# zju3dv/pvnet

Measured on NVIDIA H100. Metric: images/sec (480x640, K=9) backbone+vote, higher is better.
Workload: dtype tf32 (fp32 storage, fp32 accumulate; vote fp32/fp64)

## Files before the change

pvnet_b200/csrc/conv_col.cu:

```cuda
#include "conv_tc.cuh"
#include "ptx.cuh"

#include <cstdlib>
#include <mutex>
#include <new>

namespace pvnet {

int g_conv_mode = 0;

namespace {

constexpr int COL_TH = 16, COL_TW = 8;
constexpr int COL_THREADS = 384;
constexpr int HEAD_MAX = 64;

__host__ __device__ constexpr int head_pitch(int hc) { return hc <= 8 ? 8 : (hc <= 24 ? 24 : 40); }
constexpr int HEAD_CPITCH = COL_TH * COL_TW + 4;
__host__ __device__ constexpr int head_stage_floats(int hc)
{
    return COL_TH * COL_TW * head_pitch(hc) > hc * HEAD_CPITCH ? COL_TH * COL_TW * head_pitch(hc) : hc * HEAD_CPITCH;
}
__host__ __device__ constexpr int head_stage_bytes(int hc) { return (head_stage_floats(hc) * 4 + COL_TH * COL_TW + 127) & ~127; }

struct ColGeom {
    int Ho, Wo, tiles_x, tiles_y, total_tiles;
    int cin_chunks, cin_pad;
    int split_chunk;
    int pad_l, pad_t;
    int stages;
    int resident;
    int out_cs, out_co, res_cs, res_co;
    int act, round_out;
    int head_cout, head_seg, mask_esz;
    int head_nhwc;
};

__device__ __forceinline__ void head_store_tile(const ColGeom &g, uint32_t sv, uint32_t sm, float *head_out, void *mask,
                                                int img, int y0, int x0, int tid, int nthr)
{
    const int hc = g.head_cout, pp = head_pitch(hc);
    const int nx = min(COL_TW, g.Wo - x0), ny = min(COL_TH, g.Ho - y0);
    const size_t npix = (size_t)g.Ho * g.Wo;
    const bool vec = (reinterpret_cast<uintptr_t>(head_out) & 15) == 0 && (g.head_nhwc ? hc % 4 == 0 : g.Wo % 4 == 0);
    for (int u = tid; u < 32 * hc; u += nthr) {
        if (g.head_nhwc) {
            const int r = u / (2 * hc), e0 = 4 * (u - r * 2 * hc);
            if (r >= ny) continue;
            float *dst = head_out + (((size_t)img * g.Ho + y0 + r) * g.Wo + x0) * hc + e0;
            if (vec) {
                const int col = e0 / hc;
                if (col < nx)
                    *reinterpret_cast<float4 *>(dst) = ptx::lds128(sv + 4u * (uint32_t)((r * COL_TW + col) * pp + e0 - col * hc));
            } else {
#pragma unroll
                for (int i = 0; i < 4; ++i) {
                    const int col = (e0 + i) / hc;
                    if (col < nx) dst[i] = ptx::lds32(sv + 4u * (uint32_t)((r * COL_TW + col) * pp + e0 + i - col * hc));
                }
            }
        } else {
            const int co = u >> 5, r = (u >> 1) & 15, xo = 4 * (u & 1);
            if (r >= ny) continue;
            float *dst = head_out + ((size_t)img * hc + co) * npix + (size_t)(y0 + r) * g.Wo + x0 + xo;
            const uint32_t src = sv + 4u * (uint32_t)(co * HEAD_CPITCH + r * COL_TW + xo);
            if (vec) {
                if (xo < nx) *reinterpret_cast<float4 *>(dst) = ptx::lds128(src);
            } else {
#pragma unroll
                for (int i = 0; i < 4; ++i)
                    if (xo + i < nx) dst[i] = ptx::lds32(src + 4u * i);
            }
        }
    }
    if (!mask) return;
    for (int p = tid; p < COL_TH * COL_TW; p += nthr) {
        const int r = p / COL_TW, c = p % COL_TW;
        if (r >= ny || c >= nx) continue;
        const size_t pix = ((size_t)img * g.Ho + y0 + r) * g.Wo + x0 + c;
        const uint32_t v = ptx::lds8(sm + (uint32_t)p);
        if (g.mask_esz == 8) reinterpret_cast<long long *>(mask)[pix] = v;
        else reinterpret_cast<unsigned char *>(mask)[pix] = (unsigned char)v;
    }
}

template <int KC, bool HEAD, int KH, int BN, bool WIDE = false>
__global__ void __launch_bounds__(COL_THREADS, 1)
    k_conv_col(const __grid_constant__ CUtensorMap tmA, const __grid_constant__ CUtensorMap tmA2,
               const __grid_constant__ CUtensorMap tmB, const __grid_constant__ CUtensorMap tmBw, const __grid_constant__ ColGeom g,
               const float *__restrict__ bias, const float *__restrict__ res, float *__restrict__ out,
               const float *__restrict__ head_w, const float *__restrict__ head_b, float *__restrict__ head_out,
               void *__restrict__ mask)
{
    static_assert(!HEAD || BN == 32, "fused head: 32 input channels");
    static_assert(!HEAD || KC == 8, "fused head: convraw.0's 8-channel chunks");
    static_assert((KC == 16) == (KH == 4), "16-channel chunks are the 4x4 stem's, and only its");
    static_assert(!WIDE || (HEAD && KC == 8 && KH == 3), "wide first source: convraw.0 form only");
    constexpr int ROWB = KC * 4;
    constexpr int B_TILE = BN * ROWB;
    constexpr int PITCH = COL_TW + KH - 1;
    constexpr int A_BOX = (COL_TH + KH - 1) * PITCH * ROWB;
    constexpr int A_BYTES = (A_BOX + 1023) & ~1023;
    constexpr int WIDE_BOX = (COL_TH + KH - 1) * PITCH * 128;
    constexpr int WIDE_BYTES = (WIDE_BOX + 1023) & ~1023;
    extern __shared__ uint8_t smem_raw[];
    uint8_t *smem = reinterpret_cast<uint8_t *>((reinterpret_cast<uintptr_t>(smem_raw) + 1023) & ~uintptr_t(1023));
    const int n_btiles = KH * KH * g.cin_chunks;
    const int n_loads = WIDE ? 2 : g.cin_chunks;
    const int stage_bytes = WIDE ? WIDE_BYTES : A_BYTES + (g.resident ? 0 : KH * KH * B_TILE);
    uint8_t *sB = smem;
    uint8_t *sA = smem + (g.resident ? (size_t)n_btiles * B_TILE : 0);
    uint8_t *sH = sA + (size_t)g.stages * stage_bytes;
    uint8_t *sHS = sH + (HEAD ? 4096 : 0);
    const int hs_bytes = HEAD ? head_stage_bytes(g.head_cout) : 0;
    uint64_t *wfull = reinterpret_cast<uint64_t *>(sHS + 2 * hs_bytes);
    uint64_t *full = wfull + 1;
    uint64_t *empty = full + g.stages;
    uint64_t *hstaged = empty + g.stages;
    uint64_t *hfree = hstaged + 2;
    float *s_bias = reinterpret_cast<float *>(empty + g.stages + (HEAD ? 4 : 0));
    float *s_head = s_bias + 64;
    constexpr int STORE_THREADS = 96;

    const int warp = threadIdx.x >> 5, lane = threadIdx.x & 31;
    if (threadIdx.x == 0) {
        ptx::mbar_init(wfull, 1);
        for (int s = 0; s < g.stages; ++s) {
            ptx::mbar_init(&full[s], 1);
            ptx::mbar_init(&empty[s], 8);
        }
        if (HEAD)
            for (int b = 0; b < 2; ++b) {
                ptx::mbar_init(&hstaged[b], 256);
                ptx::mbar_init(&hfree[b], STORE_THREADS);
            }
        ptx::fence_barrier_init();
    }
    for (int i = threadIdx.x; i < BN; i += blockDim.x) s_bias[i] = bias[i];
    if (HEAD) {
        for (int i = threadIdx.x; i < 32; i += blockDim.x) s_head[i] = i < g.head_cout ? head_b[i] : 0.f;
        for (int i = threadIdx.x; i < 32 * 32; i += blockDim.x) {
            const int n = i >> 5, p = i & 31, q = p & 7;
            const int k = (p & ~7) + (q < 4 ? 2 * q : 2 * (q - 4) + 1);
            const float v = n < g.head_cout ? head_w[n * 32 + k] : 0.f;
            *reinterpret_cast<float *>(sH + ptx::swizzle_off((uint32_t)(n * 128 + p * 4), 128)) = v;
        }
        ptx::fence_proxy_async();
    }
    __syncthreads();
    const int tiles_per_img = g.tiles_x * g.tiles_y;

    if (warp >= 8) {
        const int pw = warp - 8;
        if (pw == 0 && lane == 0 && g.resident) {
            ptx::mbar_arrive_expect_tx(wfull, (uint32_t)(n_btiles * B_TILE));
            for (int cc = WIDE ? g.split_chunk : 0; cc < g.cin_chunks; ++cc)
                for (int t = 0; t < KH * KH; ++t)
                    ptx::tma_load_2d(sB + (size_t)(cc * KH * KH + t) * B_TILE, &tmB, wfull, t * g.cin_pad + cc * KC, 0);
            if (WIDE)
                for (int t = 0; t < KH * KH; ++t) ptx::tma_load_2d(sB + (size_t)t * BN * 128, &tmBw, wfull, t * g.cin_pad, 0);
        }
        if (HEAD && pw != 0) {
            const int tid = threadIdx.x - 9 * 32;
            int it = 0;
            for (int tile = blockIdx.x; tile < g.total_tiles; tile += gridDim.x, ++it) {
                const int b = it & 1;
                const int img = tile / tiles_per_img;
                const int trem = tile - img * tiles_per_img;
                const int tyi = trem / g.tiles_x, txi = trem - tyi * g.tiles_x;
                const uint32_t buf = ptx::smem_u32(sHS) + (uint32_t)(b * hs_bytes);
                ptx::mbar_wait(&hstaged[b], (uint32_t)(it >> 1) & 1u);
                head_store_tile(g, buf, buf + 4u * (uint32_t)head_stage_floats(g.head_cout), head_out, mask, img, tyi * COL_TH,
                                txi * COL_TW, tid, STORE_THREADS);
                ptx::mbar_arrive(&hfree[b]);
            }
            return;
        }
        if (pw != 0) return;
        int s = 0;
        uint32_t ph = 0;
        const uint32_t tx_bytes = (uint32_t)(A_BOX + (g.resident ? 0 : KH * KH * B_TILE));
        for (int tile = blockIdx.x; tile < g.total_tiles; tile += gridDim.x) {
            const int img = tile / tiles_per_img;
            const int trem = tile - img * tiles_per_img;
            const int tyi = trem / g.tiles_x, txi = trem - tyi * g.tiles_x;
            const int y0 = tyi * COL_TH, x0 = txi * COL_TW;
            for (int cc = 0; cc < n_loads; ++cc) {
                uint8_t *st = sA + (size_t)s * stage_bytes;
                if (WIDE) {
                    if (pw == 0 && lane == 0) {
                        ptx::mbar_wait(&empty[s], ph ^ 1u);
                        ptx::mbar_arrive_expect_tx(&full[s], (uint32_t)(cc == 0 ? WIDE_BOX : A_BOX));
                        ptx::tma_load_4d(st, cc == 0 ? &tmA : &tmA2, &full[s], 0, x0 - g.pad_l, y0 - g.pad_t, img);
                    }
                    __syncwarp();
                } else if (pw == 0) {
                    if (lane == 0) {
                        ptx::mbar_wait(&empty[s], ph ^ 1u);
                        ptx::mbar_arrive_expect_tx(&full[s], tx_bytes);
                        if (cc < g.split_chunk)
                            ptx::tma_load_4d(st, &tmA, &full[s], cc * KC, x0 - g.pad_l, y0 - g.pad_t, img);
                        else
                            ptx::tma_load_4d(st, &tmA2, &full[s], (cc - g.split_chunk) * KC, x0 - g.pad_l, y0 - g.pad_t, img);
                        if (!g.resident)
                            for (int t = 0; t < KH * KH; ++t)
                                ptx::tma_load_2d(st + A_BYTES + (size_t)t * B_TILE, &tmB, &full[s], t * g.cin_pad + cc * KC, 0);
                    }
                    __syncwarp();
                }
                if (++s == g.stages) {
                    s = 0;
                    ph ^= 1u;
                }
            }
        }
        return;
    }

    const int wg = warp >> 2, wq = warp & 3;
    const int g8 = lane >> 2, t4 = lane & 3;
    const uint32_t sA_u = ptx::smem_u32(sA), sB_u = ptx::smem_u32(sB);
    if (g.resident) ptx::mbar_wait(wfull, 0);
    int s = 0;
    uint32_t ph = 0;
    int it = 0;
    for (int tile = blockIdx.x; tile < g.total_tiles; tile += gridDim.x, ++it) {
        float acc[BN / 2];
#pragma unroll
        for (int i = 0; i < BN / 2; ++i) acc[i] = 0.f;
        int prev = -1;
        for (int cc = 0; cc < n_loads; ++cc) {
            ptx::mbar_wait(&full[s], ph);
            const uint32_t a0 = sA_u + (uint32_t)s * (uint32_t)stage_bytes;
            ptx::wgmma_fence();
            if (WIDE && cc == 0) {
                const uint64_t ad0 = ptx::make_kmajor_desc(a0 + (uint32_t)(8 * wg * PITCH * 128), 128, PITCH * 128);
                const uint64_t bd0 = ptx::make_kmajor_desc(sB_u, 128);
#pragma unroll
                for (int ks = 0; ks < 4; ++ks)
#pragma unroll
                    for (int t = 0; t < KH * KH; ++t)
                        ptx::Wgmma<BN>::ss(acc, ad0 + (uint64_t)(((t / KH) * PITCH + t % KH) * 128 / 16 + 2 * ks),
                                           bd0 + (uint64_t)(t * (BN * 128) / 16 + 2 * ks), (t | ks) != 0 ? 1u : 0u);
            } else {
                const int c8 = WIDE ? g.split_chunk : cc;
                const uint32_t b0 = g.resident ? sB_u + (uint32_t)(c8 * KH * KH * B_TILE) : a0 + (uint32_t)A_BYTES;
                const uint64_t ad0 = ptx::make_kmajor_desc(a0 + (uint32_t)(8 * wg * PITCH * ROWB), ROWB, PITCH * ROWB);
                const uint64_t bd0 = ptx::make_kmajor_desc(b0, ROWB);
#pragma unroll
                for (int t = 0; t < KH * KH; ++t) {
                    const uint64_t ad = ad0 + (uint64_t)(((t / KH) * PITCH + t % KH) * ROWB / 16);
                    const uint64_t bd = bd0 + (uint64_t)(t * B_TILE / 16);
#pragma unroll
                    for (int ks = 0; ks < KC / 8; ++ks)
                        ptx::Wgmma<BN>::ss(acc, ad + (uint64_t)(2 * ks), bd + (uint64_t)(2 * ks), (c8 | t | ks) != 0 ? 1u : 0u);
                }
            }
            ptx::wgmma_commit();
            ptx::wgmma_wait<1>();
            ptx::fence_regs(acc);
            if (prev >= 0 && lane == 0) ptx::mbar_arrive(&empty[prev]);
            prev = s;
            if (++s == g.stages) {
                s = 0;
                ph ^= 1u;
            }
        }
        ptx::wgmma_wait<0>();
        ptx::fence_regs(acc);
        if (lane == 0) ptx::mbar_arrive(&empty[prev]);

        const int img = tile / tiles_per_img;
        const int trem = tile - img * tiles_per_img;
        const int tyi = trem / g.tiles_x, txi = trem - tyi * g.tiles_x;
        const int ty = 8 * wg + 2 * wq;
        if constexpr (!HEAD) {
            bool ok[2];
            size_t pix[2];
#pragma unroll
            for (int h = 0; h < 2; ++h) {
                const int y = tyi * COL_TH + ty + h, x = txi * COL_TW + g8;
                ok[h] = y < g.Ho && x < g.Wo;
                pix[h] = ok[h] ? ((size_t)img * g.Ho + y) * g.Wo + x : 0;
            }
            float2 rv[2][BN / 8];
            if (res) {
#pragma unroll
                for (int h = 0; h < 2; ++h)
#pragma unroll
                    for (int j = 0; j < BN / 8; ++j)
                        rv[h][j] = ok[h] ? __ldg(reinterpret_cast<const float2 *>(res + pix[h] * g.res_cs + g.res_co + 8 * j + 2 * t4))
                                         : make_float2(0.f, 0.f);
            }
#pragma unroll
            for (int h = 0; h < 2; ++h) {
                if (!ok[h]) continue;
                float *optr = out + pix[h] * g.out_cs + g.out_co;
#pragma unroll
                for (int j = 0; j < BN / 8; ++j) {
                    const int c = 8 * j + 2 * t4;
                    float2 v = make_float2(acc[4 * j + 2 * h] + s_bias[c], acc[4 * j + 2 * h + 1] + s_bias[c + 1]);
                    if (res) {
                        v.x += rv[h][j].x;
                        v.y += rv[h][j].y;
                    }
                    v.x = epi_act(v.x, g.act, g.round_out);
                    v.y = epi_act(v.y, g.act, g.round_out);
                    *reinterpret_cast<float2 *>(optr + c) = v;
                }
            }
        } else {
            uint32_t a2[4][4];
#pragma unroll
            for (int j = 0; j < 4; ++j)
#pragma unroll
                for (int f = 0; f < 4; ++f) {
                    const int r = 4 * j + ((f & 1) << 1) + (f >> 1);
                    const int c = 8 * j + 2 * t4 + (f >> 1);
                    a2[j][f] = __float_as_uint(ptx::round_tf32(epi_act(acc[r] + s_bias[c], g.act, g.round_out)));
                }
            float hacc[16];
#pragma unroll
            for (int i = 0; i < 16; ++i) hacc[i] = 0.f;
            const uint64_t hd = ptx::make_kmajor_desc(ptx::smem_u32(sH), 128);
            ptx::wgmma_fence();
#pragma unroll
            for (int j = 0; j < 4; ++j) ptx::Wgmma<32>::rs(hacc, a2[j], hd + (uint64_t)(2 * j), j != 0 ? 1u : 0u);
            ptx::wgmma_commit();
            ptx::wgmma_wait<0>();
            ptx::fence_regs(hacc);
            const int hc = g.head_cout, pp = head_pitch(hc);
            const uint32_t sv = ptx::smem_u32(sHS) + (uint32_t)((it & 1) * hs_bytes);
            const uint32_t sm = sv + 4u * (uint32_t)head_stage_floats(hc);
            ptx::mbar_wait(&hfree[it & 1], ((uint32_t)(it >> 1) & 1u) ^ 1u);
#pragma unroll
            for (int h = 0; h < 2; ++h) {
                const uint32_t p = (uint32_t)((ty + h) * COL_TW + g8);
                float best = -INFINITY;
                int best_c = 0;
#pragma unroll
                for (int j = 0; j < 4; ++j) {
                    const int co = 8 * j + 2 * t4;
                    float val[2];
#pragma unroll
                    for (int e = 0; e < 2; ++e) {
                        val[e] = hacc[4 * j + 2 * h + e] + s_head[co + e];
                        if (co + e < g.head_seg && val[e] > best) {
                            best = val[e];
                            best_c = co + e;
                        }
                    }
                    if (co < hc) {
                        if (g.head_nhwc) {
                            ptx::sts64(sv + 4u * (p * pp + co), make_float2(val[0], val[1]));
                        } else {
                            ptx::sts32(sv + 4u * (co * HEAD_CPITCH + p), val[0]);
                            if (co + 1 < hc) ptx::sts32(sv + 4u * ((co + 1) * HEAD_CPITCH + p), val[1]);
                        }
                    }
                }
#pragma unroll
                for (int o = 1; o < 4; o <<= 1) {
                    const float ob = __shfl_xor_sync(0xffffffffu, best, o);
                    const int oc = __shfl_xor_sync(0xffffffffu, best_c, o);
                    if (ob > best || (ob == best && oc < best_c)) {
                        best = ob;
                        best_c = oc;
                    }
                }
                if (t4 == 0) ptx::sts8(sm + p, (uint32_t)best_c);
            }
            ptx::mbar_arrive(&hstaged[it & 1]);
        }
    }
}

struct ColPlan {
    CUtensorMap tmA, tmA2, tmB, tmBw;
    ColGeom g;
    int kc, ksize, head, bn, wide;
    unsigned grid;
    size_t smem;
    const float *bias, *res;
    float *out;
    HeadDesc hd;
};

constexpr size_t SMEM_LIMIT = 227 * 1024;

int col_kc(int Cin) { return Cin % 32 == 0 ? 32 : (Cin == 16 ? 16 : 8); }
int col_cin_pad(int Cin) { return Cin == 16 ? 16 : (Cin + 31) / 32 * 32; }

size_t col_smem(int kc, int ksize, int cin_chunks, int bn, int stages, bool head, bool resident)
{
    const size_t rowb = (size_t)kc * 4;
    const size_t a_box = (size_t)(COL_TH + ksize - 1) * (COL_TW + ksize - 1) * rowb;
    const size_t a = (a_box + 1023) & ~(size_t)1023, bt = (size_t)bn * rowb;
    return 1024 + (resident ? (size_t)ksize * ksize * cin_chunks * bt : 0) +
           (size_t)stages * (a + (resident ? 0 : (size_t)ksize * ksize * bt)) + (head ? 4096 : 0) +
           (size_t)(1 + 2 * stages) * 8 + (64 + 32) * 4;
}

template <int KC, bool HEAD, int KH, int BN, bool WIDE = false>
int col_launch(const ColPlan &p, cudaStream_t s)
{
    if (p.bn != BN || p.kc != KC || p.ksize != KH || p.head != (HEAD ? 1 : 0) || p.wide != (WIDE ? 1 : 0)) {
        set_error("conv(col): no kernel instantiation for this plan (Cout %d, chunk %d, ksize %d)", p.bn, p.kc, p.ksize);
        return PVNET_E_STATE;
    }
    auto fn = k_conv_col<KC, HEAD, KH, BN, WIDE>;
    const cudaError_t attr_err = ensure_max_smem((const void *)fn, (int)SMEM_LIMIT);
    PV_CUDA(attr_err);
    const HeadDesc &h = p.hd;
    fn<<<p.grid, COL_THREADS, p.smem, s>>>(p.tmA, p.tmA2, p.tmB, p.tmBw, p.g, p.bias, p.res, p.out, p.head ? h.w : nullptr,
                                           p.head ? h.bias : nullptr, p.head ? h.out_nchw : nullptr,
                                           p.head ? h.mask : nullptr);
    PV_LAUNCHED("k_conv_col");
    return PVNET_OK;
}

}

bool conv_col_eligible(const ConvDesc &d)
{
    if ((d.ksize != 3 && d.ksize != 4) || d.stride != 1 || d.dilation != 1 || d.Cout > 64 || d.Cout % 32 != 0)
        return false;
    const int cin = d.Cin + d.Cin2;
    const int kc = col_kc(cin);
    if (d.Cin % kc != 0 || d.Cin2 % kc != 0) return false;
    if ((d.ksize == 4) != (kc == 16)) return false;
    return col_smem(kc, d.ksize, (cin + kc - 1) / kc, d.Cout, 2, true, false) <= SMEM_LIMIT;
}

size_t conv_col_plan_size() { return sizeof(ColPlan); }

int conv_col_plan_at(const ConvDesc &d, const HeadDesc *head, void *storage)
{
    ColPlan *p = new (storage) ColPlan();
    PV_CHECK_ARG(conv_col_eligible(d), "conv(col): layer not eligible for the column kernel");
    PV_CHECK_ARG(d.in && d.w && d.bias && (d.out || head), "conv(col): null pointer");
    PV_CHECK_ARG(d.in_cs % 4 == 0 && d.in_co % 4 == 0 && d.out_cs % 4 == 0 && d.out_co % 4 == 0,
                 "conv(col): channel strides/offsets must be multiples of 4 floats");
    PV_CHECK_ARG(!d.res || (d.res_cs % 4 == 0 && d.res_co % 4 == 0), "conv(col): residual stride/offset alignment");
    PV_CHECK_ARG(!head || (d.Cout == 32 && col_kc(d.Cin + d.Cin2) == 8 && head->cout >= 1 && head->cout <= 32 && head->w && head->bias &&
                           head->out_nchw && (!head->mask || head->mask_esz == 1 || head->mask_esz == 8)),
                 "conv(col): bad fused-head description");
    const int kc = col_kc(d.Cin + d.Cin2);
    ColGeom &g = p->g;
    g.pad_l = g.pad_t = d.ksize == 4 ? 2 : 1;
    g.Ho = d.H;
    g.Wo = d.W;
    g.tiles_x = (d.W + COL_TW - 1) / COL_TW;
    g.tiles_y = (d.H + COL_TH - 1) / COL_TH;
    g.total_tiles = g.tiles_x * g.tiles_y * d.b;
    g.cin_chunks = (d.Cin + d.Cin2) / kc;
    g.split_chunk = d.in2 ? d.Cin / kc : g.cin_chunks;
    g.cin_pad = col_cin_pad(d.Cin + d.Cin2);
    g.out_cs = d.out_cs;
    g.out_co = d.out_co;
    g.res_cs = d.res_cs;
    g.res_co = d.res_co;
    g.act = d.act;
    g.round_out = d.round_out;
    g.head_cout = head ? head->cout : 0;
    g.head_seg = head ? head->seg_dim : 0;
    g.mask_esz = head ? head->mask_esz : 0;
    g.head_nhwc = 0;
    const bool hd = head != nullptr;
    const size_t hs = hd ? 2 * (size_t)head_stage_bytes(head->cout) + 4 * 8 : 0;
    bool wide = hd && d.in2 && d.Cin == 32 && d.Cin2 == 8 && kc == 8 && d.ksize == 3;
    const size_t wx = col_smem(32, 3, 0, 0, 1, false, false) - col_smem(8, 3, 0, 0, 1, false, false);
    int stages = 8;
    bool resident = true;
    while (stages > 2 && col_smem(kc, d.ksize, g.cin_chunks, d.Cout, stages, hd, true) + hs + (wide ? stages * wx : 0) > SMEM_LIMIT)
        --stages;
    if (col_smem(kc, d.ksize, g.cin_chunks, d.Cout, stages, hd, true) + hs + (wide ? stages * wx : 0) > SMEM_LIMIT) {
        wide = false;
        resident = false;
        stages = 8;
        while (stages > 2 && col_smem(kc, d.ksize, g.cin_chunks, d.Cout, stages, hd, false) + hs > SMEM_LIMIT) --stages;
    }
    g.stages = stages;
    g.resident = resident ? 1 : 0;
    p->smem = col_smem(kc, d.ksize, g.cin_chunks, d.Cout, stages, hd, resident) + hs + (wide ? stages * wx : 0);
    p->wide = wide ? 1 : 0;
    PV_CHECK_ARG(p->smem <= SMEM_LIMIT, "conv(col): layer does not fit in shared memory");
    p->kc = kc;
    p->ksize = d.ksize;
    p->bn = d.Cout;
    p->head = hd ? 1 : 0;
    if (head) p->hd = *head;
    {
        const float *base = d.in + d.in_co;
        cuuint64_t dims[4] = {(cuuint64_t)d.Cin, (cuuint64_t)d.W, (cuuint64_t)d.H, (cuuint64_t)d.b};
        cuuint64_t strides[3] = {(cuuint64_t)d.in_cs * 4, (cuuint64_t)d.W * d.in_cs * 4,
                                 (cuuint64_t)d.H * d.W * d.in_cs * 4};
        const int akc = wide ? 32 : kc;
        cuuint32_t box[4] = {(cuuint32_t)akc, (cuuint32_t)(COL_TW + d.ksize - 1), (cuuint32_t)(COL_TH + d.ksize - 1), 1};
        int rc = tma_encode(&p->tmA, base, 4, dims, strides, box, akc * 4);
        if (rc) return rc;
        p->tmA2 = p->tmA;
    }
    if (d.in2) {
        PV_CHECK_ARG(d.in2_cs % 4 == 0 && d.in2_co % 4 == 0 && d.Cin2 > 0, "conv(col): second source stride/offset alignment");
        cuuint64_t dims[4] = {(cuuint64_t)d.Cin2, (cuuint64_t)d.W, (cuuint64_t)d.H, (cuuint64_t)d.b};
        cuuint64_t strides[3] = {(cuuint64_t)d.in2_cs * 4, (cuuint64_t)d.W * d.in2_cs * 4,
                                 (cuuint64_t)d.H * d.W * d.in2_cs * 4};
        cuuint32_t box[4] = {(cuuint32_t)kc, (cuuint32_t)(COL_TW + d.ksize - 1), (cuuint32_t)(COL_TH + d.ksize - 1), 1};
        int rc = tma_encode(&p->tmA2, d.in2 + d.in2_co, 4, dims, strides, box, kc * 4);
        if (rc) return rc;
    }
    {
        cuuint64_t dims[2] = {(cuuint64_t)d.ksize * d.ksize * g.cin_pad, (cuuint64_t)d.Cout};
        cuuint64_t strides[1] = {(cuuint64_t)d.ksize * d.ksize * g.cin_pad * 4};
        cuuint32_t box[2] = {(cuuint32_t)kc, (cuuint32_t)d.Cout};
        int rc = tma_encode(&p->tmB, d.w, 2, dims, strides, box, kc * 4);
        if (rc) return rc;
        p->tmBw = p->tmB;
        if (wide) {
            box[0] = 32;
            if ((rc = tma_encode(&p->tmBw, d.w, 2, dims, strides, box, 128))) return rc;
        }
    }
    PV_CHECK_ARG(!head || (uintptr_t)head->w % 16 == 0, "conv(col): head weights must be 16-byte aligned");
    long long grid = (long long)sm_count();
    if (grid > g.total_tiles) grid = g.total_tiles;
    p->grid = (unsigned)grid;
    p->bias = d.bias;
    p->res = d.res;
    p->out = d.out;
    return PVNET_OK;
}

void conv_col_set_head_ptrs(void *storage, float *out_nchw, void *mask, int mask_esz, int nhwc)
{
    ColPlan *p = static_cast<ColPlan *>(storage);
    p->g.head_nhwc = nhwc;
    p->hd.out_nchw = out_nchw;
    p->hd.mask = mask;
    p->hd.mask_esz = mask_esz;
    p->g.mask_esz = mask_esz;
}

int conv_col_launch_at(const void *storage, cudaStream_t s)
{
    const ColPlan &p = *static_cast<const ColPlan *>(storage);
    if (p.wide) return col_launch<8, true, 3, 32, true>(p, s);
    if (p.head) return col_launch<8, true, 3, 32>(p, s);
    const bool n64 = p.bn == 64;
    if (p.ksize == 4) return n64 ? col_launch<16, false, 4, 64>(p, s) : col_launch<16, false, 4, 32>(p, s);
    if (p.kc == 32) return n64 ? col_launch<32, false, 3, 64>(p, s) : col_launch<32, false, 3, 32>(p, s);
    return n64 ? col_launch<8, false, 3, 64>(p, s) : col_launch<8, false, 3, 32>(p, s);
}

}

extern "C" {
int pvnet_conv_set_mode(int mode)
{
    PV_CHECK_ARG(mode >= 0 && mode <= 2, "mode must be 0, 1 or 2");
    pvnet::g_conv_mode = mode;
    return PVNET_OK;
}
}
```

Measured before the change: 1713.

## Ping-pong consumer warpgroups across tiles in non-head column conv

For non-head convolutions, each of the two consumer warpgroups now computes a whole tile (both 8-row M blocks, two accumulator sets) and the two alternate tiles. A turn barrier hands off MMA issue between them, so one warpgroup's epilogue (bias, residual, activation, stores) overlaps the other's tensor-core work. The change doubles accumulator registers per thread, which risks spills or lower occupancy for large BN. It also adds barrier bookkeeping for stage skipping.

```diff
diff --git a/pvnet_b200/csrc/conv_col.cu b/pvnet_b200/csrc/conv_col.cu
--- a/pvnet_b200/csrc/conv_col.cu
+++ b/pvnet_b200/csrc/conv_col.cu
@@ -118,22 +118,27 @@
     uint64_t *empty = full + g.stages;
     uint64_t *hstaged = empty + g.stages;
     uint64_t *hfree = hstaged + 2;
-    float *s_bias = reinterpret_cast<float *>(empty + g.stages + (HEAD ? 4 : 0));
+    uint64_t *turn = hstaged + (HEAD ? 4 : 0);
+    float *s_bias = reinterpret_cast<float *>(turn + 2);
     float *s_head = s_bias + 64;
     constexpr int STORE_THREADS = 96;
+    constexpr bool PP = !HEAD;
+    constexpr int NACC = PP ? 2 : 1;
 
     const int warp = threadIdx.x >> 5, lane = threadIdx.x & 31;
     if (threadIdx.x == 0) {
         ptx::mbar_init(wfull, 1);
         for (int s = 0; s < g.stages; ++s) {
             ptx::mbar_init(&full[s], 1);
-            ptx::mbar_init(&empty[s], 8);
+            ptx::mbar_init(&empty[s], PP ? 4 : 8);
         }
         if (HEAD)
             for (int b = 0; b < 2; ++b) {
                 ptx::mbar_init(&hstaged[b], 256);
                 ptx::mbar_init(&hfree[b], STORE_THREADS);
             }
+        if (PP)
+            for (int b = 0; b < 2; ++b) ptx::mbar_init(&turn[b], 4);
         ptx::fence_barrier_init();
     }
     for (int i = threadIdx.x; i < BN; i += blockDim.x) s_bias[i] = bias[i];
@@ -223,90 +228,118 @@
     if (g.resident) ptx::mbar_wait(wfull, 0);
     int s = 0;
     uint32_t ph = 0;
-    int it = 0;
-    for (int tile = blockIdx.x; tile < g.total_tiles; tile += gridDim.x, ++it) {
-        float acc[BN / 2];
-#pragma unroll
-        for (int i = 0; i < BN / 2; ++i) acc[i] = 0.f;
+    auto advance = [&](int n) {
+        for (int i = 0; i < n; ++i)
+            if (++s == g.stages) {
+                s = 0;
+                ph ^= 1u;
+            }
+    };
+    if (PP && wg == 1) advance(n_loads);
+    const int mb0 = PP ? 0 : wg;
+    int it = PP ? wg : 0;
+    for (int tile = blockIdx.x + (PP ? wg : 0) * gridDim.x; tile < g.total_tiles;
+         tile += (PP ? 2 : 1) * gridDim.x, it += PP ? 2 : 1) {
+        float acc[NACC][BN / 2];
+#pragma unroll
+        for (int m = 0; m < NACC; ++m)
+#pragma unroll
+            for (int i = 0; i < BN / 2; ++i) acc[m][i] = 0.f;
+        if (PP && it > 0) ptx::mbar_wait(&turn[wg], (uint32_t)((it - 1) >> 1) & 1u);
         int prev = -1;
         for (int cc = 0; cc < n_loads; ++cc) {
             ptx::mbar_wait(&full[s], ph);
             const uint32_t a0 = sA_u + (uint32_t)s * (uint32_t)stage_bytes;
             ptx::wgmma_fence();
             if (WIDE && cc == 0) {
-                const uint64_t ad0 = ptx::make_kmajor_desc(a0 + (uint32_t)(8 * wg * PITCH * 128), 128, PITCH * 128);
+                uint64_t ad0[NACC];
+#pragma unroll
+                for (int m = 0; m < NACC; ++m)
+                    ad0[m] = ptx::make_kmajor_desc(a0 + (uint32_t)(8 * (mb0 + m) * PITCH * 128), 128, PITCH * 128);
                 const uint64_t bd0 = ptx::make_kmajor_desc(sB_u, 128);
 #pragma unroll
                 for (int ks = 0; ks < 4; ++ks)
 #pragma unroll
                     for (int t = 0; t < KH * KH; ++t)
-                        ptx::Wgmma<BN>::ss(acc, ad0 + (uint64_t)(((t / KH) * PITCH + t % KH) * 128 / 16 + 2 * ks),
-                                           bd0 + (uint64_t)(t * (BN * 128) / 16 + 2 * ks), (t | ks) != 0 ? 1u : 0u);
+#pragma unroll
+                        for (int m = 0; m < NACC; ++m)
+                            ptx::Wgmma<BN>::ss(acc[m], ad0[m] + (uint64_t)(((t / KH) * PITCH + t % KH) * 128 / 16 + 2 * ks),
+                                               bd0 + (uint64_t)(t * (BN * 128) / 16 + 2 * ks), (t | ks) != 0 ? 1u : 0u);
             } else {
                 const int c8 = WIDE ? g.split_chunk : cc;
                 const uint32_t b0 = g.resident ? sB_u + (uint32_t)(c8 * KH * KH * B_TILE) : a0 + (uint32_t)A_BYTES;
-                const uint64_t ad0 = ptx::make_kmajor_desc(a0 + (uint32_t)(8 * wg * PITCH * ROWB), ROWB, PITCH * ROWB);
+                uint64_t ad0[NACC];
+#pragma unroll
+                for (int m = 0; m < NACC; ++m)
+                    ad0[m] = ptx::make_kmajor_desc(a0 + (uint32_t)(8 * (mb0 + m) * PITCH * ROWB), ROWB, PITCH * ROWB);
                 const uint64_t bd0 = ptx::make_kmajor_desc(b0, ROWB);
 #pragma unroll
                 for (int t = 0; t < KH * KH; ++t) {
-                    const uint64_t ad = ad0 + (uint64_t)(((t / KH) * PITCH + t % KH) * ROWB / 16);
+                    const uint64_t toff = (uint64_t)(((t / KH) * PITCH + t % KH) * ROWB / 16);
                     const uint64_t bd = bd0 + (uint64_t)(t * B_TILE / 16);
 #pragma unroll
                     for (int ks = 0; ks < KC / 8; ++ks)
-                        ptx::Wgmma<BN>::ss(acc, ad + (uint64_t)(2 * ks), bd + (uint64_t)(2 * ks), (c8 | t | ks) != 0 ? 1u : 0u);
+#pragma unroll
+                        for (int m = 0; m < NACC; ++m)
+                            ptx::Wgmma<BN>::ss(acc[m], ad0[m] + toff + (uint64_t)(2 * ks), bd + (uint64_t)(2 * ks),
+                                               (c8 | t | ks) != 0 ? 1u : 0u);
                 }
             }
             ptx::wgmma_commit();
+            if (PP && cc == n_loads - 1 && lane == 0) ptx::mbar_arrive(&turn[wg ^ 1]);
             ptx::wgmma_wait<1>();
-            ptx::fence_regs(acc);
+#pragma unroll
+            for (int m = 0; m < NACC; ++m) ptx::fence_regs(acc[m]);
             if (prev >= 0 && lane == 0) ptx::mbar_arrive(&empty[prev]);
             prev = s;
-            if (++s == g.stages) {
-                s = 0;
-                ph ^= 1u;
-            }
+            advance(1);
         }
         ptx::wgmma_wait<0>();
-        ptx::fence_regs(acc);
+#pragma unroll
+        for (int m = 0; m < NACC; ++m) ptx::fence_regs(acc[m]);
         if (lane == 0) ptx::mbar_arrive(&empty[prev]);
+        if (PP) advance(n_loads);
 
         const int img = tile / tiles_per_img;
         const int trem = tile - img * tiles_per_img;
         const int tyi = trem / g.tiles_x, txi = trem - tyi * g.tiles_x;
-        const int ty = 8 * wg + 2 * wq;
         if constexpr (!HEAD) {
-            bool ok[2];
-            size_t pix[2];
-#pragma unroll
-            for (int h = 0; h < 2; ++h) {
-                const int y = tyi * COL_TH + ty + h, x = txi * COL_TW + g8;
-                ok[h] = y < g.Ho && x < g.Wo;
-                pix[h] = ok[h] ? ((size_t)img * g.Ho + y) * g.Wo + x : 0;
-            }
-            float2 rv[2][BN / 8];
-            if (res) {
-#pragma unroll
-                for (int h = 0; h < 2; ++h)
-#pragma unroll
-                    for (int j = 0; j < BN / 8; ++j)
-                        rv[h][j] = ok[h] ? __ldg(reinterpret_cast<const float2 *>(res + pix[h] * g.res_cs + g.res_co + 8 * j + 2 * t4))
-                                         : make_float2(0.f, 0.f);
-            }
-#pragma unroll
-            for (int h = 0; h < 2; ++h) {
-                if (!ok[h]) continue;
-                float *optr = out + pix[h] * g.out_cs + g.out_co;
-#pragma unroll
-                for (int j = 0; j < BN / 8; ++j) {
-                    const int c = 8 * j + 2 * t4;
-                    float2 v = make_float2(acc[4 * j + 2 * h] + s_bias[c], acc[4 * j + 2 * h + 1] + s_bias[c + 1]);
-                    if (res) {
-                        v.x += rv[h][j].x;
-                        v.y += rv[h][j].y;
+#pragma unroll
+            for (int m = 0; m < NACC; ++m) {
+                const int ty = 8 * (mb0 + m) + 2 * wq;
+                bool ok[2];
+                size_t pix[2];
+#pragma unroll
+                for (int h = 0; h < 2; ++h) {
+                    const int y = tyi * COL_TH + ty + h, x = txi * COL_TW + g8;
+                    ok[h] = y < g.Ho && x < g.Wo;
+                    pix[h] = ok[h] ? ((size_t)img * g.Ho + y) * g.Wo + x : 0;
+                }
+                float2 rv[2][BN / 8];
+                if (res) {
+#pragma unroll
+                    for (int h = 0; h < 2; ++h)
+#pragma unroll
+                        for (int j = 0; j < BN / 8; ++j)
+                            rv[h][j] = ok[h] ? __ldg(reinterpret_cast<const float2 *>(res + pix[h] * g.res_cs + g.res_co + 8 * j + 2 * t4))
+                                             : make_float2(0.f, 0.f);
+                }
+#pragma unroll
+                for (int h = 0; h < 2; ++h) {
+                    if (!ok[h]) continue;
+                    float *optr = out + pix[h] * g.out_cs + g.out_co;
+#pragma unroll
+                    for (int j = 0; j < BN / 8; ++j) {
+                        const int c = 8 * j + 2 * t4;
+                        float2 v = make_float2(acc[m][4 * j + 2 * h] + s_bias[c], acc[m][4 * j + 2 * h + 1] + s_bias[c + 1]);
+                        if (res) {
+                            v.x += rv[h][j].x;
+                            v.y += rv[h][j].y;
+                        }
+                        v.x = epi_act(v.x, g.act, g.round_out);
+                        v.y = epi_act(v.y, g.act, g.round_out);
+                        *reinterpret_cast<float2 *>(optr + c) = v;
                     }
-                    v.x = epi_act(v.x, g.act, g.round_out);
-                    v.y = epi_act(v.y, g.act, g.round_out);
-                    *reinterpret_cast<float2 *>(optr + c) = v;
                 }
             }
         } else {
@@ -317,7 +350,7 @@
                 for (int f = 0; f < 4; ++f) {
                     const int r = 4 * j + ((f & 1) << 1) + (f >> 1);
                     const int c = 8 * j + 2 * t4 + (f >> 1);
-                    a2[j][f] = __float_as_uint(ptx::round_tf32(epi_act(acc[r] + s_bias[c], g.act, g.round_out)));
+                    a2[j][f] = __float_as_uint(ptx::round_tf32(epi_act(acc[0][r] + s_bias[c], g.act, g.round_out)));
                 }
             float hacc[16];
 #pragma unroll
@@ -335,7 +368,7 @@
             ptx::mbar_wait(&hfree[it & 1], ((uint32_t)(it >> 1) & 1u) ^ 1u);
 #pragma unroll
             for (int h = 0; h < 2; ++h) {
-                const uint32_t p = (uint32_t)((ty + h) * COL_TW + g8);
+                const uint32_t p = (uint32_t)((8 * wg + 2 * wq + h) * COL_TW + g8);
                 float best = -INFINITY;
                 int best_c = 0;
 #pragma unroll
@@ -398,7 +431,7 @@
     const size_t a = (a_box + 1023) & ~(size_t)1023, bt = (size_t)bn * rowb;
     return 1024 + (resident ? (size_t)ksize * ksize * cin_chunks * bt : 0) +
            (size_t)stages * (a + (resident ? 0 : (size_t)ksize * ksize * bt)) + (head ? 4096 : 0) +
-           (size_t)(1 + 2 * stages) * 8 + (64 + 32) * 4;
+           (size_t)(3 + 2 * stages) * 8 + (64 + 32) * 4;
 }
 
 template <int KC, bool HEAD, int KH, int BN, bool WIDE = false>
```

Result: no change. 1729, median of 6 (+0.9%).
